# TobiasDeBruijn/UU-INFOGR-Raytracer

Hardware: AMD Instinct MI355X
Metric: Mray/s (primary+shadow+reflect) and fps at 1920×1080, 1/2/4/8 MI355X (higher is better)
Workload: dtype f32

## Files before the change

uu-infogr-raytracer_amd/csrc/rt_internal.h:

```cpp
#pragma once
#include <stdint.h>

#include "rt_resolve.h"

namespace rtk {

struct DevSphere {
    float cx, cy, cz, r2;
};

enum : uint32_t { MAT_MIRROR = 1u, MAT_DIFFUSE = 2u, MAT_SPEC = 4u, MAT_DARK_OK = 8u };

enum : uint32_t { POW_GENERIC = 0u, POW_ONE = 1u, POW_HALF = 2u, POW_TWO = 3u };

struct DevMaterial {
    float kd[3];
    float amb[3];
    float ks[3];
    float n;
    float km[3];
    uint32_t flags;
    uint32_t pow_kind;
    uint32_t pad;
};
// ... 80 lines not shown

struct CopyJob {
    const int32_t* src;
    int32_t* dst;
    unsigned long long words;
    unsigned long long dst_stride;
    unsigned band_words;
    unsigned pad;
};

struct alignas(16) DevView {
    float cam[3], right[3], up[3], fwd[3];
    int prim_const;
    int mbox_n;
    int mbox_plane[2];
    float mbox_tmax[2];
    int pad[2];
    PrimConst pc[MAX_PRIM_CONST];
    PrimBox pbox[MAX_PRIM_CONST];
    PrimBox mbox[2][CULL_MIN_SPHERES];
};
static_assert(sizeof(DevView) % 16 == 0, "DevView records are 16-byte aligned in their device table");

struct LaunchParams {
    const DevSphere* sph;
    const DevMaterial* mat;
    const DevPlane* pl;
    const DevLight* li;
    const DevSphereCull* scull;
    const DevShadowCull* shcull;
    const DevShadowCull* shpre;
    const DevShadowGrid* shg;
    const unsigned long long* shgrid;
    const unsigned long long* shslab;
    const DevCluster* clus;
    const float* lxt;
    const float* lyt;
    int S, P, L, limit;
    int lights_a2_ok;
    int n_clus;
    float cam[3], right[3], up[3], fwd[3];
    float pw, ph, nearc;
    int W, H;
    int band_rows, band_first, band_step, local_rows;
    int n_frames;
    int32_t* out;
    unsigned long long out_frame_bytes;
    int out_fmt;
    unsigned char* enc_wire;
    uint32_t* enc_stage;
    int enc_tiles_x, enc_tpf, enc_frame0;
    unsigned long long* counters;
    CopyJob copy;
    int copy_z;
    int prim_const;
    PrimConst pc[MAX_PRIM_CONST];
    PrimBox pbox[MAX_PRIM_CONST];
    int row_order_n;
    int col_major;
    uint16_t row_order[ROW_ORDER_MAX];
    const uint32_t* tile_order;
    uint32_t* tile_cost;
    int ss_log2;
    int mbox_n;
    int mbox_plane[2];
    float mbox_tmax[2];
    PrimBox mbox[2][CULL_MIN_SPHERES];
    const DevView* views;
    int shutter_log2;
    int adapt_thr;
    int foot_n;
    PlaneFoot foot[FOOT_MAX];
    ResolveSum* prog_acc;
    int prog_first;
    int prog_n;
    int prog_pass[2];
    int uniform_plane;
    const DevShadowGroups* shgrp;
    unsigned long long scene_stride;
    int view_ss;
};
constexpr int MIRROR_BOX_PLANES = 2;
constexpr int SINGLE_WPG = 4;
static_assert(sizeof(LaunchParams) < 4096, "LaunchParams is passed by value as the kernarg block (< 4 KiB)");

constexpr int OUT_TILES = 3;

constexpr int DIRECT_SMAX = 8;

enum : int { TV_DIRECT = 0, TV_BUNDLE = 1 };
enum : int { TM_PLAIN = 0, TM_STATS = 1, TM_TILES = 2, TM_SS = 3, TM_PATH = 4, TM_SHUTTER = 5, TM_ADAPT = 6, TM_PROG = 7, TM_ANIM = 8,
             TM_PATH_SS = 9, TM_SHUTTER_SS = 10, TM_ANIM_SS = 11 };
struct TraceVariant {
    int family;
    int gpow;
    int mode;
    int cls;
    int K;
    int wpg;
    int tord;
};

enum : unsigned { VF_GPOW = 1u, VF_STATS = 2u, VF_TILES = 4u, VF_SS = 8u, VF_PATH = 16u, VF_SHUTTER = 32u, VF_ADAPT = 64u, VF_PROG = 128u };
constexpr unsigned VF_ANIM = 1u << 18;
// ... 102 lines not shown
```

uu-infogr-raytracer_amd/csrc/rt_kernel.hip:

```cpp
#include <hip/hip_runtime.h>

#include "rt_fastmath.h"
#include "rt_codec_common.h"
#include "rt_dark.h"
#include "rt_foot.h"
#include "rt_internal.h"
#include "rt_pow.h"
#include "rt_prims.h"
#include "rt_resolve.h"
#include "rt_shadow_pre.h"

constexpr int WG_THREADS = 64, TILE_W = 8, TILE_H = 8;

namespace rtk {

constexpr unsigned COPY_WAVES = 512;
__device__ __forceinline__ size_t band_dst(const CopyJob& j, unsigned i) {
    if (j.band_words == 0) return i;
    const unsigned k = i / j.band_words;
    return (size_t)k * j.dst_stride + (i - k * j.band_words);
}
__device__ __forceinline__ void copy_job(const CopyJob& j, size_t wg, size_t nwg) {
    const size_t lane = threadIdx.x & 63;
    const unsigned long long n = j.words, n4 = n / 4;
// ... 7 lines not shown
            d4[i] = a;
            d4[i + step] = b;
            d4[i + 2 * step] = c;
            d4[i + 3 * step] = d;
        }
        for (; i < n4; i += step) d4[i] = s4[i];
    } else {
        int4* __restrict__ d4 = (int4*)j.dst;
        const unsigned bq = j.band_words / 4, sq = (unsigned)(j.dst_stride / 4);
        for (unsigned c = (unsigned)i; c < (unsigned)n4; c += (unsigned)step) {
            const unsigned k = c / bq;
            d4[k * sq + (c - k * bq)] = s4[c];
        }
    }
    if (wg == 0 && lane < n - n4 * 4) j.dst[band_dst(j, (unsigned)(n4 * 4 + lane))] = j.src[n4 * 4 + lane];
}
__device__ __forceinline__ void copy_slice(const LaunchParams& p) {
    const size_t nwg = min((size_t)gridDim.x * gridDim.y, (size_t)COPY_WAVES);
    const size_t wg = (size_t)blockIdx.y * gridDim.x + blockIdx.x;
    if (wg < nwg) copy_job(p.copy, wg, nwg);
}
__global__ __launch_bounds__(64) void band_copy_kernel(CopyJob j) { copy_job(j, blockIdx.x, gridDim.x); }

__device__ __forceinline__ void store_at(const LaunchParams& p, size_t i, uint32_t px32) {
    unsigned char* base = (unsigned char*)p.out + (size_t)blockIdx.z * p.out_frame_bytes;
    if (p.out_fmt != 1) {
        ((int32_t*)base)[i] = (int32_t)px32;
    } else {
        unsigned char* o = base + i * 3;
        o[0] = (unsigned char)px32;
        o[1] = (unsigned char)(px32 >> 8);
        o[2] = (unsigned char)(px32 >> 16);
    }
}
__device__ __forceinline__ void store_pixel(const LaunchParams& p, int r, int y, int x, uint32_t px32) {
    store_at(p, (size_t)(p.out_fmt == 2 ? y : r) * (size_t)p.W + (size_t)x, px32);
}

template <int CTRL>
__device__ __forceinline__ ResolveSum resolve_add_dpp(ResolveSum v) {
    return resolve_add(v, ResolveSum{(uint32_t)__builtin_amdgcn_update_dpp(0, (int)v.rb, CTRL, 0xf, 0xf, false),
                                     (uint32_t)__builtin_amdgcn_update_dpp(0, (int)v.g, CTRL, 0xf, 0xf, false)});
}
template <int PATTERN>
__device__ __forceinline__ ResolveSum resolve_add_swizzle(ResolveSum v) {
    return resolve_add(v, ResolveSum{(uint32_t)__builtin_amdgcn_ds_swizzle((int)v.rb, PATTERN),
                                     (uint32_t)__builtin_amdgcn_ds_swizzle((int)v.g, PATTERN)});
}
__device__ __forceinline__ ResolveSum resolve_block_sum(ResolveSum v, int s) {
    v = resolve_add_dpp<0xb1>(v);
    v = resolve_add_dpp<0x128>(v);
    if (s >= 2) {
        v = resolve_add_dpp<0x4e>(v);
        v = resolve_add_swizzle<0x401f>(v);
    }
    if (s >= 3) {
        v = resolve_add_swizzle<0x101f>(v);
        v = resolve_add(v, ResolveSum{(uint32_t)__shfl_xor((int)v.rb, 32, 64), (uint32_t)__shfl_xor((int)v.g, 32, 64)});
// ... 90 lines not shown
        if constexpr (PATH != VIEW_ARGS) return v().pc;
        else return p.pc;
    }
    __device__ __forceinline__ const PrimBox* pbox() const {
        if constexpr (PATH != VIEW_ARGS) return v().pbox;
        else return p.pbox;
    }
    __device__ __forceinline__ int mbox_n() const {
        if constexpr (PATH != VIEW_ARGS) return v().mbox_n;
        else return p.mbox_n;
    }
    __device__ __forceinline__ int mbox_plane(int k) const {
        if constexpr (PATH != VIEW_ARGS) return v().mbox_plane[k];
        else return p.mbox_plane[k];
    }
    __device__ __forceinline__ float mbox_tmax(int k) const {
        if constexpr (PATH != VIEW_ARGS) return v().mbox_tmax[k];
        else return p.mbox_tmax[k];
    }
    __device__ __forceinline__ const PrimBox* mbox(int k) const {
        if constexpr (PATH != VIEW_ARGS) return v().mbox[k];
        else return p.mbox[k];
    }
    __device__ __forceinline__ int foot_n() const {
        if constexpr (PATH != VIEW_ARGS) return -1;
        else return p.foot_n;
    }
};

template <int PATH>
struct SceneOf {
    template <bool NULLABLE, typename T>
    static __device__ __forceinline__ const T* at(const LaunchParams& p, const T* q) {
        if constexpr (PATH == VIEW_ANIM) {
            const T* z = (const T*)((const char*)q + (size_t)blockIdx.z * (size_t)p.scene_stride);
            if constexpr (NULLABLE) return q == nullptr ? nullptr : z;
            else return z;
        } else {
            return q;
        }
    }
    static __device__ __forceinline__ const DevSphere* sph(const LaunchParams& p) { return at<false>(p, p.sph); }
    static __device__ __forceinline__ const DevMaterial* mat(const LaunchParams& p) { return at<false>(p, p.mat); }
    static __device__ __forceinline__ const DevPlane* pl(const LaunchParams& p) { return at<false>(p, p.pl); }
    static __device__ __forceinline__ const DevLight* li(const LaunchParams& p) { return at<false>(p, p.li); }
    static __device__ __forceinline__ const DevSphereCull* scull(const LaunchParams& p) { return at<false>(p, p.scull); }
    static __device__ __forceinline__ const DevShadowCull* shcull(const LaunchParams& p) { return at<true>(p, p.shcull); }
    static __device__ __forceinline__ const DevShadowCull* shpre(const LaunchParams& p) { return at<true>(p, p.shpre); }
    static __device__ __forceinline__ const DevShadowGrid* shg(const LaunchParams& p) { return at<true>(p, p.shg); }
    static __device__ __forceinline__ const unsigned long long* shgrid(const LaunchParams& p) { return at<true>(p, p.shgrid); }
// ... 140 lines not shown
    static constexpr int smax = SMAX;
    unsigned s = 0, pl = 0, sh = 0;
    int lvl = 0, sel_cat = 0, sel_lvl = -1;
    __device__ __forceinline__ void sphere(bool c) { s += (!RT_SHADOW_CAT && (RT_SLOT_TALLY || c)) ? 1u : 0u; }
    __device__ __forceinline__ void shadow_sphere(bool c) {
        s += (!RT_SHADOW_CAT && (RT_SLOT_TALLY == 1 || c)) ? 1u : 0u;
    }
    __device__ __forceinline__ void plane(bool c) { pl += c ? 1u : 0u; }
    __device__ __forceinline__ void shadow(bool c) { sh += c ? 1u : 0u; }
    __device__ __forceinline__ void init(const LaunchParams& p) {
        sel_cat = p.enc_frame0 / 16;
        sel_lvl = p.enc_frame0 % 16 - 1;
    }
    __device__ __forceinline__ void set_level(int l) { lvl = l; }
    __device__ __forceinline__ void shadow_cat(int cat, unsigned n) {
        s += (RT_SHADOW_CAT && cat + 1 == sel_cat && (sel_lvl < 0 || lvl == sel_lvl)) ? n : 0u;
    }
    __device__ __forceinline__ void shadow_masks(int cat, unsigned long long m) {
        if (RT_SHADOW_CAT && cat + 1 == sel_cat && (sel_lvl < 0 || lvl == sel_lvl) && (threadIdx.x & 63) == 0)
            s += (unsigned)__builtin_popcountll(m);
    }
};

template <bool ST, int PATH = VIEW_ARGS, int SM>
__device__ __forceinline__ void add_counters(const LaunchParams& p, int lane, unsigned n_refl, unsigned n_shadow,
                                             const Tally<ST, SM>& tl) {
    if ((!PATH && blockIdx.z != (unsigned)p.copy_z) || p.counters == nullptr) return;
    const unsigned long long nf = !PATH && p.n_frames > 1 ? (unsigned long long)p.n_frames : 1ull;
    const unsigned b = wave_count(n_refl), c = wave_count(n_shadow);
    const unsigned slot = (blockIdx.y * gridDim.x + blockIdx.x) % COUNTER_SLOTS;
    unsigned long long* q = &p.counters[slot * COUNTER_STRIDE];
    if (lane == 0) {
        if (b) atomicAdd(q + CNT_REFLECT, b * nf);
        if (c) atomicAdd(q + CNT_SHADOW, c * nf);
    }
    if constexpr (ST) {
        const unsigned s = wave_count(tl.s), pl = wave_count(tl.pl), sh = wave_count(tl.sh);
        if (lane == 0) {
            if (sh) atomicAdd(q + CNT_SHADOW_RUN, sh * nf);
            if (s) atomicAdd(q + CNT_SPHERE_RUN, s * nf);
            if (pl) atomicAdd(q + CNT_PLANE_RUN, pl * nf);
        }
    }
}

#ifndef RT_UNIFORM_PLANE
#define RT_UNIFORM_PLANE 1
#endif
// ... 126 lines not shown
                tl.shadow(true);
                blocked = l_ok ? shadow_scan<true, GROUPS, PATH>(p, hp, l, li, tl) : shadow_scan<false, false, PATH>(p, hp, l, li, tl);
            }
            const float inten = blocked ? 0.0f : l.intensity;
            const float ia = inten * att;
            f3 term = mul(mk(ia, ia, ia), ph);
            if (!is_sphere) {
                term = mul(term, mk(tile, tile, tile));
                term = mk(nmax0(term.x), nmax0(term.y), nmax0(term.z));
            }
            col = add(col, term);
        }
    }
    if (flags & MAT_DIFFUSE) *n_shadow += (unsigned)p.L << CNT_SHADOW_SHIFT;
    return add(col, mk(m.amb[0], m.amb[1], m.amb[2]));
}

template <int PATH, typename T>
__device__ __forceinline__ f3 shade_plane_uniform(const LaunchParams& p, int plane, f3 hp, f3 d, float t, f3 sec,
                                                  unsigned* n_shadow, T& tl) {
    return shade_direct<false, RT_SHADOW_GROUPS != 0, PATH>(p, false, plane, hp, d, t, sec, n_shadow, tl);
}

__device__ __forceinline__ unsigned long long box_mask(const LaunchParams& p, const PrimBox* tab, int x, int y) {
    const int x_lo = __builtin_amdgcn_readlane(x, 0), x_hi = __builtin_amdgcn_readlane(x, 63);
    const int y_lo = __builtin_amdgcn_readlane(y, 0), y_hi = __builtin_amdgcn_readlane(y, 63);
    const int lane = threadIdx.x & 63;
    const bool in = lane < p.S;
    const PrimBox b = tab[in ? lane : 0];
    const bool cand = in & (b.x0 <= x_hi) & (b.x1 >= x_lo) & (b.y0 <= y_hi) & (b.y1 >= y_lo);
    return __builtin_amdgcn_ballot_w64(cand);
}
template <int PATH = VIEW_ARGS>
__device__ __forceinline__ unsigned long long prim_box_mask(const LaunchParams& p, int x, int y, int rec = 0) {
    return box_mask(p, ViewOf<PATH>{p, rec}.pbox(), x, y);
}
template <int PATH = VIEW_ARGS>
__device__ __forceinline__ unsigned mirror_box_masks(const LaunchParams& p, int x, int y, int rec = 0) {
    const ViewOf<PATH> vw{p, rec};
    unsigned m = 0;
    if (vw.mbox_n() > 0) {
        m = (unsigned)box_mask(p, vw.mbox(0), x, y);
        if (vw.mbox_n() > 1) m |= (unsigned)box_mask(p, vw.mbox(1), x, y) << 16;
    }
    return m;
}
template <int PATH = VIEW_ARGS>
__device__ __forceinline__ unsigned mirror_box_select(const LaunchParams& p, unsigned masks, float t, int prim, int rec = 0) {
    const ViewOf<PATH> vw{p, rec};
    const int pi = ~prim;
    const bool on0 = prim < 0 && pi == vw.mbox_plane(0) && t <= vw.mbox_tmax(0);
    const bool on1 = prim < 0 && pi == vw.mbox_plane(1) && t <= vw.mbox_tmax(1);
    if (__builtin_amdgcn_ballot_w64(!(on0 || on1)) != 0) return ~0u;
    unsigned m = 0;
    if (__builtin_amdgcn_ballot_w64(on0) != 0) m |= masks & 0xffffu;
    if (__builtin_amdgcn_ballot_w64(on1) != 0) m |= masks >> 16;
    return m;
}

struct TilePixel {
    int x, r, y;
    bool valid;
    float lx, ly;
};
template <bool SS = false>
__device__ __forceinline__ TilePixel tile_pixel(const LaunchParams& p, int x, int r) {
    TilePixel t;
    t.x = x, t.r = r;
    if (p.band_rows >= p.local_rows) {
        t.y = p.band_first * p.band_rows + r;
    } else if (!SS && p.band_rows == 8) {
        t.y = (p.band_first + (r >> 3) * p.band_step) * 8 + (r & 7);
    } else if (SS && (p.band_rows & (p.band_rows - 1)) == 0) {
        const int sh = 31 - __builtin_clz((unsigned)p.band_rows);
        t.y = ((p.band_first + (r >> sh) * p.band_step) << sh) + (r & (p.band_rows - 1));
    } else {
        const int band = p.band_first + (r / p.band_rows) * p.band_step;
        t.y = band * p.band_rows + (r % p.band_rows);
    }
    t.valid = x < p.W && r < p.local_rows && t.y < p.H;
    const float lx = p.lxt[t.valid ? x : 0], ly = p.lyt[t.valid ? t.y : 0];
    t.lx = t.valid ? lx : 0.0f, t.ly = t.valid ? ly : 0.0f;
    return t;
}
__device__ __forceinline__ TilePixel sample_pixel(const LaunchParams& p, int tile_x, int tile_y, int lane, int pass) {
    const int x = tile_x * TILE_W + (lane & 7), r = tile_y * TILE_H + (lane >> 3), s2 = p.ss_log2;
    return tile_pixel<true>(p, (x << s2) | (pass & ((1 << s2) - 1)), (r << s2) | (pass >> s2));
}

template <bool PRIMARY, bool A2OK, bool GATED, int PATH, typename T>
__device__ __forceinline__ void nearest_spheres(const LaunchParams& p, f3 o, f3 d, float a2, float a4, bool a2_ok,
                                                unsigned long long pmask, float& best_s, int& win_s, T& tl, int rec = 0) {
    if (PRIMARY && ViewOf<PATH>{p, rec}.prim_const()) {
        for (unsigned long long m = pmask; m;) {
            const int i = (int)__builtin_ctzll(m);
            m &= ~(1ull << i);
            tl.sphere(true);
            const PrimConst pc = ViewOf<PATH>{p, rec}.pc()[i];
            const float b = 2.0f * dot(mk(pc.ocx, pc.ocy, pc.ocz), d);
            const float disc = b * b - a4 * pc.c;
            const float t = A2OK ? root_t1(b, disc, a2) : (a2_ok ? root_t1(b, disc, a2) : root_full(b, disc, a2));
            take_primary(t, i, best_s, win_s);
        }
    } else {
        for_sphere_pairs<T>(p, [&](int i) {
            if constexpr (GATED) {
                if ((((unsigned)pmask >> i) & 3u) == 0) return;
            }
            tl.sphere(true);
            tl.sphere(i + 1 < p.S);
// ... 37 lines not shown
template <int PATH, typename T>
__device__ __forceinline__ Hit terminal_direct(const LaunchParams& p, f3 o, f3 d, T& tl) {
    float best_p = __builtin_inff();
    int win_p = -1;
    for (int i = 0; i < p.P; ++i) {
        tl.plane(true);
        plane_take(o, d, SceneOf<PATH>::pl(p)[i], i, best_p, win_p);
    }
    if (win_p < 0 || !(best_p - 0.01f > 0.0f)) return Hit{0.0f, HIT_NONE};
    const float a = dot(d, d);
    const float a2 = 2.0f * a, a4 = 4.0f * a;
    const bool a2_ok = a2 > 0.0f && a2 < __builtin_inff();
    float best_s = __builtin_inff();
    int win_s = -1;
    if (__builtin_amdgcn_ballot_w64(!a2_ok) == 0)
        nearest_spheres<false, true, false, PATH>(p, o, d, a2, a4, a2_ok, 0, best_s, win_s, tl);
    else
        nearest_spheres<false, false, false, PATH>(p, o, d, a2, a4, a2_ok, 0, best_s, win_s, tl);
    if (best_s < best_p) return Hit{0.0f, HIT_NONE};
    return Hit{best_p, ~win_p};
}

template <int PATH>
__device__ __forceinline__ bool sky_tile(const LaunchParams& p, const TilePixel& t, unsigned long long pmask, int rec) {
    const ViewOf<PATH> vw{p, rec};
    const int n = vw.foot_n();
    if (n < 0 || pmask != 0 || !vw.prim_const()) return false;
    bool may = false;
#pragma unroll
    for (int i = 0; i < FOOT_MAX; ++i) {
        if (i >= n) break;
        may |= foot_may_hit(p.foot[i], t.lx, t.ly);
    }
    return __builtin_amdgcn_ballot_w64(t.valid && may) == 0;
}

constexpr unsigned VF_TILE = ~(vf_wpg(15) | vf_tord(3));

struct TileOut {
    unsigned cnt;
    uint32_t px32;
};

template <int K, unsigned V, bool UNIFORM_OK = true, typename T>
__device__ __forceinline__ TileOut trace_tile_direct(const LaunchParams& p, int tile_x, int tile_y, float2* stk_lv,
                                                     float* stk_dv, T& tl, int rec = 0) {
    constexpr bool GPOW = (V & VF_GPOW) != 0, TILES = (V & VF_TILES) != 0, SS = ss_of(V), SHUTTER = shutter_of(V);
    constexpr bool ADAPT = (V & VF_ADAPT) != 0;
    constexpr int PATH = view_of(V);
    constexpr bool UNIFORM = RT_UNIFORM_PLANE && UNIFORM_OK && !GPOW;
    const int lane = threadIdx.x & 63;
    const TilePixel tpx = ADAPT ? sample_pixel(p, tile_x, tile_y, lane, rec)
                                : tile_pixel<SS>(p, tile_x * TILE_W + (lane & 7), tile_y * TILE_H + (lane >> 3));
    const int x = tpx.x, r = tpx.r, y = tpx.y;
    const bool valid = tpx.valid;
    const ViewOf<PATH> vw{p, rec};
    const unsigned long long pmask = vw.prim_const() ? prim_box_mask<PATH>(p, x, y, rec) : 0;
    const bool sky = sky_tile<PATH>(p, tpx, pmask, rec);
    unsigned mmask = 0;
    if constexpr (K > 1) {
        if (!sky) mmask = mirror_box_masks<PATH>(p, x, y, rec);
    }

    unsigned cnt = 0;
    typename StackFor<K>::type stk(stk_lv, stk_dv);
    f3 leaf = mk(0.0f, 0.0f, 0.0f);
    uint32_t px32 = 0;
    if (valid) {
        if (!sky) {
            const f3 cam = vw.cam();
            const float lx = tpx.lx, ly = tpx.ly, lz = 1.0f * p.nearc;
            const f3 vp = add(add(add(cam, scale(vw.right(), lx)), scale(vw.up(), ly)), scale(vw.fwd(), lz));
            f3 d = normalize(sub(vp, cam));
            f3 o = cam;

            stk.origin(d);
            Hit h = nearest_direct<true, false, PATH>(p, o, d, tl, pmask, rec);
            int count = 0;
            for (;;) {
                if (h.prim == HIT_NONE) break;
                if (h.t - 0.01f <= 0.0f) break;
                const bool is_sphere = h.prim >= 0;
                if (count > p.limit) {
                    if (!is_sphere) leaf = mk(1.0f, 1.0f, 1.0f);
// ... 24 lines not shown
                    const int code0 = __builtin_amdgcn_readlane(code, (int)__builtin_ctzll(m0));
                    if (code0 < 0 && __builtin_amdgcn_ballot_w64(rec0 && code != code0) == 0) floor_n = 1;
                }
            }
            f3 col = leaf;
            while (stk.n > floor_n) {
                float4 ra, rb;
                stk.template pop<PATH>(p, ra, rb, rec);
                const int code = __float_as_int(rb.w);
                const bool is_s = code >= 0;
                col = shade_direct<GPOW, false, PATH>(p, is_s, is_s ? code : ~code, mk(ra.x, ra.y, ra.z),
                                               mk(rb.x, rb.y, rb.z), ra.w, col, &cnt, tl);
            }
            if constexpr (UNIFORM) {
                if (floor_n != 0 && stk.n != 0) {
                    float4 ra, rb;
                    stk.template level0<PATH>(p, ra, rb, rec);
                    const int plane = ~__builtin_amdgcn_readfirstlane(__float_as_int(rb.w));
                    col = shade_plane_uniform<PATH>(p, plane, mk(ra.x, ra.y, ra.z), mk(rb.x, rb.y, rb.z), ra.w, col, &cnt, tl);
                }
            }
            px32 = (shift_channel(col.x) << 16) | (shift_channel(col.y) << 8) | shift_channel(col.z);
        }
        if constexpr (!TILES && !SS && !SHUTTER && !ADAPT) store_pixel(p, r, y, x, px32);
    }
    if constexpr (TILES) encode_tile_fused(p, px32, valid);
    if constexpr (SS && !SHUTTER) resolve_tile(p, r, y, x, valid, px32);
    return TileOut{cnt, px32};
}

template <bool SS, typename F>
__device__ __forceinline__ void shutter_tile(const LaunchParams& p, int tile_x, int tile_y, F trace) {
    const int t = p.shutter_log2, m = 1 << t;
    const int rec0 = (int)(blockIdx.z << t);
    const bool counting = p.counters != nullptr;
    ResolveSum acc{0u, 0u};
    unsigned long long n_refl = 0, n_shadow = 0;
#pragma unroll 1
    for (int s = 0; s < m; ++s) {
        int tx = tile_x, ty = tile_y;
        asm("" : "+s"(tx), "+s"(ty) : "s"(s));
        const __attribute__((address_space(4))) LaunchParams* kp =
            (const __attribute__((address_space(4))) LaunchParams*)__builtin_amdgcn_kernarg_segment_ptr();
        asm("" : "+s"(kp) : "s"(s));
        const TileOut o = trace(*(const LaunchParams*)kp, rec0 | s, tx, ty);
        acc = resolve_add(acc, resolve_unpack(o.px32));
        if (counting) {
            n_refl += wave_count(o.cnt & CNT_REFL_MASK);
            n_shadow += wave_count(o.cnt >> CNT_SHADOW_SHIFT);
        }
    }
// ... 91 lines not shown
        uint2* a = (uint2*)(p.prog_acc + ((size_t)(t.r >> s2) * wo + xo));
        if (p.prog_first > 0) {
            const uint2 before = *a;
            acc = resolve_add(acc, ResolveSum{before.x, before.y});
        }
        if (p.prog_n > 0) *a = make_uint2(acc.rb, acc.g);
        store_at(p, (size_t)((p.out_fmt == 2 ? t.y : t.r) >> s2) * wo + xo, resolve_round_div(acc, p.prog_first + p.prog_n));
    }
    if (p.counters != nullptr && blockIdx.z == (unsigned)p.copy_z && ln == 0) {
        unsigned long long* c = &p.counters[((blockIdx.y * gridDim.x + blockIdx.x) % COUNTER_SLOTS) * COUNTER_STRIDE];
        if (n_refl) atomicAdd(c + CNT_REFLECT, (unsigned long long)n_refl);
        if (n_shadow) atomicAdd(c + CNT_SHADOW, n_shadow);
    }
}

template <int K, unsigned V>
__device__ __forceinline__ void direct_kernel_body(const LaunchParams& p) {
    constexpr bool STATS = (V & VF_STATS) != 0, SHUTTER = shutter_of(V);
    constexpr int PATH = view_of(V);
    constexpr int SMAX = vf_cls_of(V), WPG = vf_wpg_of(V), TORD = vf_tord_of(V);
    constexpr int LDS_LEVELS = StackFor<K>::lds_levels;
    __shared__ float2 stk_lv[LDS_LEVELS > 0 ? LDS_LEVELS * WG_THREADS * WPG : 1];
    __shared__ float stk_dv[LDS_LEVELS > 0 ? 3 * WG_THREADS * WPG : 1];
    if (WPG == 1 && blockIdx.z < (unsigned)p.copy_z) {
        copy_slice(p);
        return;
    }
    Tally<STATS, SMAX> tl;
    const int wave = WPG > 1 && TORD != 0 ? __builtin_amdgcn_readfirstlane((int)(threadIdx.x >> 6))
                     : WPG > 1                ? (int)(threadIdx.x >> 6)
                                              : 0;
    float2* lv = stk_lv + (LDS_LEVELS > 0 ? wave * LDS_LEVELS * WG_THREADS : 0);
    float* dv = stk_dv + (LDS_LEVELS > 0 ? wave * 3 * WG_THREADS : 0);
    const bool cm = WPG > 1 && p.col_major;
    const int gx = cm ? (int)blockIdx.y : (int)blockIdx.x, gy = cm ? (int)blockIdx.x : (int)blockIdx.y;
    int tile_x = gx * WPG + wave, tile_y = WPG > 1 && gy < p.row_order_n ? (int)p.row_order[gy] : gy;
    if constexpr (TORD == 1) {
        const uint32_t t = p.tile_order[blockIdx.x * WPG + wave];
        tile_x = (int)(t & 0xffffu), tile_y = (int)(t >> 16);
    }
    struct TileRec {
        unsigned* slot;
        unsigned t0;
    };
    __shared__ TileRec t_rec[TORD == 2 ? WPG : 1];
    if (TORD == 2 && (threadIdx.x & 63) == 0) {
        const unsigned tiles_x = (unsigned)(p.W + TILE_W - 1) / TILE_W, tiles_y = (unsigned)(p.H + TILE_H - 1) / TILE_H;
        const bool in = p.tile_cost != nullptr && (unsigned)tile_x < tiles_x && (unsigned)tile_y < tiles_y;
        t_rec[wave] = TileRec{in ? p.tile_cost + ((unsigned)tile_y * tiles_x + (unsigned)tile_x) : nullptr,
                              in ? (unsigned)__builtin_amdgcn_s_memrealtime() : 0u};
    }
    if constexpr (SHUTTER) {
        shutter_tile<ss_of(V)>(p, tile_x, tile_y, [&](const LaunchParams& q, int rec, int tx, int ty) { return trace_tile_direct<K, V & VF_TILE>(q, tx, ty, lv, dv, tl, rec); });
        return;
    }
    if constexpr ((V & VF_ADAPT) != 0) {
        adaptive_tile(p, tile_x, tile_y, [&](const LaunchParams& q, int pass, int tx, int ty) { return trace_tile_direct<K, V & VF_TILE>(q, tx, ty, lv, dv, tl, pass); });
        return;
    }
    if constexpr ((V & VF_PROG) != 0) {
        progressive_tile(p, tile_x, tile_y, [&](const LaunchParams& q, int pass, int tx, int ty) { return trace_tile_direct<K, ((V & VF_TILE) & ~VF_PROG) | VF_ADAPT>(q, tx, ty, lv, dv, tl, pass); });
        return;
    }
    const unsigned cnt = trace_tile_direct<K, V & VF_TILE, TORD != 2>(p, tile_x, tile_y, lv, dv, tl).cnt;
    add_counters<STATS, PATH>(p, threadIdx.x & 63, cnt & CNT_REFL_MASK, cnt >> CNT_SHADOW_SHIFT, tl);
    if (TORD == 2 && (threadIdx.x & 63) == 0) {
        const TileRec r = t_rec[threadIdx.x >> 6];
        if (r.slot != nullptr) *r.slot = (unsigned)__builtin_amdgcn_s_memrealtime() - r.t0;
    }
}
template <int K, unsigned V>
__global__ __launch_bounds__(WG_THREADS * vf_wpg_of(V)) __attribute__((amdgpu_num_sgpr(80))) void trace_direct_kernel(LaunchParams p) {
    static_assert(!(V & VF_GPOW), "GPOW variants run trace_direct_kernel_gpow");
    direct_kernel_body<K, V>(p);
}
template <int K, unsigned V>
__global__ __launch_bounds__(WG_THREADS * vf_wpg_of(V)) void trace_direct_kernel_gpow(LaunchParams p) {
    static_assert((V & VF_GPOW) != 0, "variants without GPOW run trace_direct_kernel");
    direct_kernel_body<K, V>(p);
}

struct Bundle {
    f3 O, A;
    float R, delta;
    bool ok;
    bool any;
};

__device__ __forceinline__ float readlane_f(float v, int lane) {
    return __int_as_float(__builtin_amdgcn_readlane(__float_as_int(v), lane));
}
__device__ __forceinline__ f3 readlane3(f3 v, int lane) {
    return mk(readlane_f(v.x, lane), readlane_f(v.y, lane), readlane_f(v.z, lane));
}
template <int CTRL>
// ... 462 lines not shown
        float4 ra = make_float4(0.0f, 0.0f, 0.0f, 1.0f), rb = make_float4(0.0f, 0.0f, 1.0f, 0.0f);
        if (act) stk.template pop<PATH>(p, ra, rb, rec);
        const unsigned long long am = __builtin_amdgcn_ballot_w64(act);
        if (am != ~0ull) {
            const int ref = __builtin_ctzll(am);
            const float4 qa = make_float4(readlane_f(ra.x, ref), readlane_f(ra.y, ref), readlane_f(ra.z, ref),
                                          readlane_f(ra.w, ref));
            const float4 qb = make_float4(readlane_f(rb.x, ref), readlane_f(rb.y, ref), readlane_f(rb.z, ref),
                                          readlane_f(rb.w, ref));
            if (!act) {
                ra = qa;
                rb = qb;
            }
        }
        const int code = __float_as_int(rb.w);
        const bool is_s = code >= 0;
        tl.set_level(level);
        col = shade_bundle<GPOW, MERGED, PATH>(p, act, is_s, is_s ? code : ~code, mk(ra.x, ra.y, ra.z), mk(rb.x, rb.y, rb.z),
                                         ra.w, col, cnt, tl, level);
    }
    return col;
}

template <int K, unsigned V, typename T>
__device__ __forceinline__ TileOut trace_tile_bundle(const LaunchParams& p, int tile_x, int tile_y, float2* stk_lv,
                                                     float* stk_dv, T& tl, int rec = 0) {
    constexpr bool GPOW = (V & VF_GPOW) != 0, TILES = (V & VF_TILES) != 0, SS = ss_of(V), SHUTTER = shutter_of(V);
    constexpr bool ADAPT = (V & VF_ADAPT) != 0;
    constexpr int PATH = view_of(V);
    constexpr int MERGED = vf_cls_of(V);
    const int lane = threadIdx.x & 63;
    const TilePixel tpx = ADAPT ? sample_pixel(p, tile_x, tile_y, lane, rec)
                                : tile_pixel<SS>(p, tile_x * TILE_W + (lane & 7), tile_y * TILE_H + (lane >> 3));
    const int x = tpx.x, y = tpx.y;
    const bool valid = tpx.valid;

    unsigned cnt = 0;
    const ViewOf<PATH> vw{p, rec};
    const f3 cam = vw.cam();
    const float lx = tpx.lx, ly = tpx.ly, lz = 1.0f * p.nearc;
    const f3 vp = add(add(add(cam, scale(vw.right(), lx)), scale(vw.up(), ly)), scale(vw.fwd(), lz));
    f3 d = normalize(sub(vp, cam));
    f3 o = cam;

    typename StackFor<K>::type stk(stk_lv, stk_dv);
    stk.origin(d);
    f3 leaf = mk(0.0f, 0.0f, 0.0f);
    bool active = valid;
    const unsigned long long pmask = vw.prim_const() ? prim_box_mask<PATH>(p, x, y, rec) : 0;
    Hit h = nearest_bundle<true, PATH>(p, o, d, active, tl, pmask, nullptr, rec);
    for (int count = 0;; ++count) {
        if (active) {
            const bool is_sphere = h.prim >= 0;
            if (h.prim == HIT_NONE || h.t - 0.01f <= 0.0f) {
                active = false;
            } else if (count > p.limit) {
                if (!is_sphere) leaf = mk(1.0f, 1.0f, 1.0f);
                active = false;
            } else {
                const f3 hp = add(o, scale(d, h.t));
                stk.push(make_float4(hp.x, hp.y, hp.z, h.t), make_float4(d.x, d.y, d.z, __int_as_float(h.prim)));
                const int prim = is_sphere ? h.prim : ~h.prim;
                const uint32_t flags = SceneOf<PATH>::mat(p)[is_sphere ? prim : p.S + prim].flags;
                if (!(flags & MAT_MIRROR)) {
                    active = false;
                } else {
                    o = reflect_at<PATH>(p, o, d, h.t, h.prim);
                    ++cnt;
                }
            }
        }
        if (__builtin_amdgcn_ballot_w64(active) == 0) break;
// ... 16 lines not shown
        }
    }

    const f3 col = fold_converged<GPOW, MERGED, PATH>(p, stk, leaf, &cnt, tl, rec);
    const uint32_t px32 = (shift_channel(col.x) << 16) | (shift_channel(col.y) << 8) | shift_channel(col.z);
    if constexpr (TILES) encode_tile_fused(p, px32, valid);
    else if constexpr (!SHUTTER && !ADAPT) {
        const int ln = (int)__builtin_amdgcn_mbcnt_hi(~0u, __builtin_amdgcn_mbcnt_lo(~0u, 0u));
        const TilePixel q = tile_pixel<SS>(p, tile_x * TILE_W + (ln & 7), tile_y * TILE_H + (ln >> 3));
        if constexpr (SS) resolve_tile(p, q.r, q.y, q.x, q.valid, px32);
        else if (q.valid) store_pixel(p, q.r, q.y, q.x, px32);
    }
    return TileOut{cnt, px32};
}

template <int K, unsigned V>
__device__ __forceinline__ void bundle_kernel_body(const LaunchParams& p) {
    constexpr bool STATS = (V & VF_STATS) != 0, SHUTTER = shutter_of(V);
    constexpr int PATH = view_of(V);
    constexpr int TORD = vf_tord_of(V);
    constexpr int LDS_LEVELS = StackFor<K>::lds_levels;
    __shared__ float2 stk_lv[LDS_LEVELS > 0 ? LDS_LEVELS * WG_THREADS : 1];
    __shared__ float stk_dv[LDS_LEVELS > 0 ? 3 * WG_THREADS : 1];
    if (blockIdx.z < (unsigned)p.copy_z) {
        copy_slice(p);
        return;
    }
    Tally<STATS> tl;
    tl.init(p);
    int tile_x = (int)blockIdx.x, tile_y = (int)blockIdx.y;
    if constexpr (TORD == 1) {
        const uint32_t t = p.tile_order[blockIdx.y * gridDim.x + blockIdx.x];
        tile_x = (int)(t & 0xffffu), tile_y = (int)(t >> 16);
    }
    struct TileRec {
        unsigned* slot;
        unsigned t0;
    };
    __shared__ TileRec t_rec[1];
    if (TORD == 2 && (threadIdx.x & 63) == 0)
        t_rec[0] = TileRec{blockIdx.z == (unsigned)p.copy_z ? p.tile_cost + (blockIdx.y * gridDim.x + blockIdx.x) : nullptr,
                           (unsigned)__builtin_amdgcn_s_memrealtime()};
    if constexpr (SHUTTER) {
        shutter_tile<ss_of(V)>(p, tile_x, tile_y, [&](const LaunchParams& q, int rec, int tx, int ty) { return trace_tile_bundle<K, V & VF_TILE>(q, tx, ty, stk_lv, stk_dv, tl, rec); });
        return;
    }
    if constexpr ((V & VF_ADAPT) != 0) {
        adaptive_tile(p, tile_x, tile_y, [&](const LaunchParams& q, int pass, int tx, int ty) { return trace_tile_bundle<K, V & VF_TILE>(q, tx, ty, stk_lv, stk_dv, tl, pass); });
        return;
    }
    if constexpr ((V & VF_PROG) != 0) {
        progressive_tile(p, tile_x, tile_y, [&](const LaunchParams& q, int pass, int tx, int ty) { return trace_tile_bundle<K, ((V & VF_TILE) & ~VF_PROG) | VF_ADAPT>(q, tx, ty, stk_lv, stk_dv, tl, pass); });
        return;
    }
    const unsigned cnt = trace_tile_bundle<K, V & VF_TILE>(p, tile_x, tile_y, stk_lv, stk_dv, tl).cnt;
    add_counters<STATS, PATH>(p, threadIdx.x & 63, cnt & CNT_REFL_MASK, cnt >> CNT_SHADOW_SHIFT, tl);
    if (TORD == 2 && (threadIdx.x & 63) == 0 && t_rec[0].slot != nullptr)
        *t_rec[0].slot = (unsigned)__builtin_amdgcn_s_memrealtime() - t_rec[0].t0;
}
template <int K, unsigned V>
__global__ __launch_bounds__(WG_THREADS, 8) __attribute__((amdgpu_num_sgpr(80))) void trace_bundle_kernel(
    LaunchParams p) {
    static_assert(!(V & VF_GPOW), "GPOW variants run trace_bundle_kernel_gpow");
    bundle_kernel_body<K, V>(p);
}
template <int K, unsigned V>
__global__ __launch_bounds__(WG_THREADS) void trace_bundle_kernel_gpow(LaunchParams p) {
    static_assert((V & VF_GPOW) != 0, "variants without GPOW run trace_bundle_kernel");
    bundle_kernel_body<K, V>(p);
}

__device__ __forceinline__ void append_segment(DevSegment* out, int cap, unsigned* count, f3 o, f3 e, int kind,
                                               int pixel) {
    const unsigned i = atomicAdd(count, 1u);
    if (i < (unsigned)cap) out[i] = DevSegment{o.x, o.y, o.z, e.x, e.y, e.z, kind, pixel};
}

__global__ __launch_bounds__(256) void debug_segments_kernel(LaunchParams p, int stride, DevSegment* out, int cap,
// ... 178 lines not shown
```

Baseline: 305,700.

## Reorder kernel arguments into cache-line head and batch early scalar loads

Reorders LaunchParams so the per-wave scalars read at kernel entry (dimensions, band layout, counts, footprints) sit together in two 64-byte lines at offset 0, with the output tail grouped into one line. It also adds load_head and wave_tables helpers that pull these fields and the per-lane box tables into registers together at the start, using empty asm pins to keep them in SGPRs and VGPRs. The goal is fewer scattered, serialized kernarg scalar loads and an earlier issue of the lxt/lyt and box loads. In exchange it raises register pressure under the 80-SGPR cap, and it adds an optional tail path that is off by default.

```diff
diff --git a/uu-infogr-raytracer_amd/csrc/rt_internal.h b/uu-infogr-raytracer_amd/csrc/rt_internal.h
--- a/uu-infogr-raytracer_amd/csrc/rt_internal.h
+++ b/uu-infogr-raytracer_amd/csrc/rt_internal.h
@@ -1,5 +1,7 @@
 #pragma once
 #include <stdint.h>
+
+#include <type_traits>
 
 #include "rt_resolve.h"
 
@@ -126,7 +128,43 @@
 };
 static_assert(sizeof(DevView) % 16 == 0, "DevView records are 16-byte aligned in their device table");
 
-struct LaunchParams {
+struct alignas(64) LaunchHead {
+    const float* lxt;
+    const float* lyt;
+    int W, H;
+    int band_rows, band_first, band_step, local_rows;
+    int ss_log2;
+    int copy_z;
+    int prim_const;
+    int S;
+    int foot_n;
+    int mbox_n;
+    int P, L, limit;
+    int uniform_plane;
+    int mbox_plane[2];
+    float mbox_tmax[2];
+    const DevView* views;
+    int row_order_n;
+    int col_major;
+    int lights_a2_ok;
+    int n_clus;
+    int head_pad[2];
+};
+static_assert(sizeof(LaunchHead) == 128 && alignof(LaunchHead) == 64, "the launch head is two 64-byte lines");
+
+struct LaunchParams : LaunchHead {
+    PlaneFoot foot[FOOT_MAX];
+    float pw, ph, nearc;
+    int tail_pad;
+    int32_t* out;
+    unsigned long long out_frame_bytes;
+    unsigned long long* counters;
+    unsigned char* enc_wire;
+    uint32_t* enc_stage;
+    int out_fmt;
+    int n_frames;
+    int enc_tiles_x, enc_tpf, enc_frame0;
+    int tail_end_pad;
     const DevSphere* sph;
     const DevMaterial* mat;
     const DevPlane* pl;
@@ -138,52 +176,46 @@
     const unsigned long long* shgrid;
     const unsigned long long* shslab;
     const DevCluster* clus;
-    const float* lxt;
-    const float* lyt;
-    int S, P, L, limit;
-    int lights_a2_ok;
-    int n_clus;
     float cam[3], right[3], up[3], fwd[3];
-    float pw, ph, nearc;
-    int W, H;
-    int band_rows, band_first, band_step, local_rows;
-    int n_frames;
-    int32_t* out;
-    unsigned long long out_frame_bytes;
-    int out_fmt;
-    unsigned char* enc_wire;
-    uint32_t* enc_stage;
-    int enc_tiles_x, enc_tpf, enc_frame0;
-    unsigned long long* counters;
     CopyJob copy;
-    int copy_z;
-    int prim_const;
     PrimConst pc[MAX_PRIM_CONST];
     PrimBox pbox[MAX_PRIM_CONST];
-    int row_order_n;
-    int col_major;
+    PrimBox mbox[2][CULL_MIN_SPHERES];
     uint16_t row_order[ROW_ORDER_MAX];
     const uint32_t* tile_order;
     uint32_t* tile_cost;
-    int ss_log2;
-    int mbox_n;
-    int mbox_plane[2];
-    float mbox_tmax[2];
-    PrimBox mbox[2][CULL_MIN_SPHERES];
-    const DevView* views;
+    int line_pad[10];
     int shutter_log2;
     int adapt_thr;
-    int foot_n;
-    PlaneFoot foot[FOOT_MAX];
     ResolveSum* prog_acc;
     int prog_first;
     int prog_n;
     int prog_pass[2];
-    int uniform_plane;
     const DevShadowGroups* shgrp;
     unsigned long long scene_stride;
     int view_ss;
 };
+static_assert(std::is_trivially_copyable<LaunchParams>::value && std::is_base_of<LaunchHead, LaunchParams>::value,
+              "LaunchParams is copied into the kernel argument segment byte for byte");
+#if defined(__clang__)
+#pragma clang diagnostic push
+#pragma clang diagnostic ignored "-Winvalid-offsetof"
+#elif defined(__GNUC__)
+#pragma GCC diagnostic push
+#pragma GCC diagnostic ignored "-Winvalid-offsetof"
+#endif
+static_assert(__builtin_offsetof(LaunchParams, view_ss) + 2 * sizeof(int) == sizeof(LaunchParams), "view_ss is the last word");
+static_assert(alignof(LaunchParams) == 64 && __builtin_offsetof(LaunchParams, lxt) == 0 &&
+                  __builtin_offsetof(LaunchParams, foot) == sizeof(LaunchHead),
+              "the launch head at offset 0, the plane footprints directly behind it");
+static_assert(__builtin_offsetof(LaunchParams, out) % 64 == 0 &&
+                  __builtin_offsetof(LaunchParams, enc_frame0) + sizeof(int) <= __builtin_offsetof(LaunchParams, out) + 64,
+              "the tail: one 64-byte line");
+#if defined(__clang__)
+#pragma clang diagnostic pop
+#elif defined(__GNUC__)
+#pragma GCC diagnostic pop
+#endif
 constexpr int MIRROR_BOX_PLANES = 2;
 constexpr int SINGLE_WPG = 4;
 static_assert(sizeof(LaunchParams) < 4096, "LaunchParams is passed by value as the kernarg block (< 4 KiB)");
diff --git a/uu-infogr-raytracer_amd/csrc/rt_kernel.hip b/uu-infogr-raytracer_amd/csrc/rt_kernel.hip
--- a/uu-infogr-raytracer_amd/csrc/rt_kernel.hip
+++ b/uu-infogr-raytracer_amd/csrc/rt_kernel.hip
@@ -53,7 +53,8 @@
 }
 __global__ __launch_bounds__(64) void band_copy_kernel(CopyJob j) { copy_job(j, blockIdx.x, gridDim.x); }
 
-__device__ __forceinline__ void store_at(const LaunchParams& p, size_t i, uint32_t px32) {
+template <typename O>
+__device__ __forceinline__ void store_at(const O& p, size_t i, uint32_t px32) {
     unsigned char* base = (unsigned char*)p.out + (size_t)blockIdx.z * p.out_frame_bytes;
     if (p.out_fmt != 1) {
         ((int32_t*)base)[i] = (int32_t)px32;
@@ -64,7 +65,8 @@
         o[2] = (unsigned char)(px32 >> 16);
     }
 }
-__device__ __forceinline__ void store_pixel(const LaunchParams& p, int r, int y, int x, uint32_t px32) {
+template <typename O>
+__device__ __forceinline__ void store_pixel(const O& p, int r, int y, int x, uint32_t px32) {
     store_at(p, (size_t)(p.out_fmt == 2 ? y : r) * (size_t)p.W + (size_t)x, px32);
 }
 
@@ -201,10 +203,6 @@
         if constexpr (PATH != VIEW_ARGS) return v().mbox[k];
         else return p.mbox[k];
     }
-    __device__ __forceinline__ int foot_n() const {
-        if constexpr (PATH != VIEW_ARGS) return -1;
-        else return p.foot_n;
-    }
 };
 
 template <int PATH>
@@ -391,8 +389,8 @@
     }
 };
 
-template <bool ST, int PATH = VIEW_ARGS, int SM>
-__device__ __forceinline__ void add_counters(const LaunchParams& p, int lane, unsigned n_refl, unsigned n_shadow,
+template <bool ST, int PATH = VIEW_ARGS, int SM, typename O>
+__device__ __forceinline__ void add_counters(const O& p, int lane, unsigned n_refl, unsigned n_shadow,
                                              const Tally<ST, SM>& tl) {
     if ((!PATH && blockIdx.z != (unsigned)p.copy_z) || p.counters == nullptr) return;
     const unsigned long long nf = !PATH && p.n_frames > 1 ? (unsigned long long)p.n_frames : 1ull;
@@ -565,26 +563,29 @@
     return shade_direct<false, RT_SHADOW_GROUPS != 0, PATH>(p, false, plane, hp, d, t, sec, n_shadow, tl);
 }
 
-__device__ __forceinline__ unsigned long long box_mask(const LaunchParams& p, const PrimBox* tab, int x, int y) {
+__device__ __forceinline__ PrimBox box_load(const PrimBox* tab, int S) {
+    const int lane = threadIdx.x & 63;
+    return tab[lane < S ? lane : 0];
+}
+__device__ __forceinline__ unsigned long long box_test(const PrimBox& b, int S, int x, int y) {
     const int x_lo = __builtin_amdgcn_readlane(x, 0), x_hi = __builtin_amdgcn_readlane(x, 63);
     const int y_lo = __builtin_amdgcn_readlane(y, 0), y_hi = __builtin_amdgcn_readlane(y, 63);
-    const int lane = threadIdx.x & 63;
-    const bool in = lane < p.S;
-    const PrimBox b = tab[in ? lane : 0];
+    const bool in = (int)(threadIdx.x & 63) < S;
     const bool cand = in & (b.x0 <= x_hi) & (b.x1 >= x_lo) & (b.y0 <= y_hi) & (b.y1 >= y_lo);
     return __builtin_amdgcn_ballot_w64(cand);
+}
+__device__ __forceinline__ unsigned long long box_mask(const LaunchHead& h, const PrimBox* tab, int x, int y) {
+    return box_test(box_load(tab, h.S), h.S, x, y);
 }
 template <int PATH = VIEW_ARGS>
 __device__ __forceinline__ unsigned long long prim_box_mask(const LaunchParams& p, int x, int y, int rec = 0) {
     return box_mask(p, ViewOf<PATH>{p, rec}.pbox(), x, y);
 }
-template <int PATH = VIEW_ARGS>
-__device__ __forceinline__ unsigned mirror_box_masks(const LaunchParams& p, int x, int y, int rec = 0) {
-    const ViewOf<PATH> vw{p, rec};
+__device__ __forceinline__ unsigned mirror_box_masks(const PrimBox& b0, const PrimBox& b1, int mbox_n, int S, int x, int y) {
     unsigned m = 0;
-    if (vw.mbox_n() > 0) {
-        m = (unsigned)box_mask(p, vw.mbox(0), x, y);
-        if (vw.mbox_n() > 1) m |= (unsigned)box_mask(p, vw.mbox(1), x, y) << 16;
+    if (mbox_n > 0) {
+        m = (unsigned)box_test(b0, S, x, y);
+        if (mbox_n > 1) m |= (unsigned)box_test(b1, S, x, y) << 16;
     }
     return m;
 }
@@ -607,7 +608,7 @@
     float lx, ly;
 };
 template <bool SS = false>
-__device__ __forceinline__ TilePixel tile_pixel(const LaunchParams& p, int x, int r) {
+__device__ __forceinline__ TilePixel tile_pixel(const LaunchHead& p, int x, int r) {
     TilePixel t;
     t.x = x, t.r = r;
     if (p.band_rows >= p.local_rows) {
@@ -622,13 +623,79 @@
         t.y = band * p.band_rows + (r % p.band_rows);
     }
     t.valid = x < p.W && r < p.local_rows && t.y < p.H;
-    const float lx = p.lxt[t.valid ? x : 0], ly = p.lyt[t.valid ? t.y : 0];
+    typedef const __attribute__((address_space(1))) float* gtab;
+    const float lx = ((gtab)p.lxt)[t.valid ? x : 0], ly = ((gtab)p.lyt)[t.valid ? t.y : 0];
     t.lx = t.valid ? lx : 0.0f, t.ly = t.valid ? ly : 0.0f;
     return t;
 }
-__device__ __forceinline__ TilePixel sample_pixel(const LaunchParams& p, int tile_x, int tile_y, int lane, int pass) {
+__device__ __forceinline__ TilePixel sample_pixel(const LaunchHead& p, int tile_x, int tile_y, int lane, int pass) {
     const int x = tile_x * TILE_W + (lane & 7), r = tile_y * TILE_H + (lane >> 3), s2 = p.ss_log2;
     return tile_pixel<true>(p, (x << s2) | (pass & ((1 << s2) - 1)), (r << s2) | (pass >> s2));
+}
+
+struct WaveHead : LaunchHead {
+    PlaneFoot foot[FOOT_MAX];
+};
+template <bool FOOT>
+__device__ __forceinline__ WaveHead load_head(int tie = 0) {
+    const __attribute__((address_space(4))) LaunchParams* kp =
+        (const __attribute__((address_space(4))) LaunchParams*)__builtin_amdgcn_kernarg_segment_ptr();
+    asm("" : "+s"(kp) : "s"(tie));
+    const LaunchParams& p = *(const LaunchParams*)kp;
+    WaveHead h;
+    static_cast<LaunchHead&>(h) = p;
+    if constexpr (FOOT) {
+#pragma unroll
+        for (int i = 0; i < FOOT_MAX; ++i) h.foot[i] = p.foot[i];
+        asm("" : "+s"(h.lxt), "+s"(h.lyt), "+s"(h.W), "+s"(h.H), "+s"(h.band_rows), "+s"(h.band_first), "+s"(h.band_step),
+                 "+s"(h.local_rows), "+s"(h.ss_log2), "+s"(h.copy_z), "+s"(h.prim_const), "+s"(h.S), "+s"(h.foot_n), "+s"(h.mbox_n),
+                 "+s"(h.foot[0].a), "+s"(h.foot[0].b), "+s"(h.foot[0].c), "+s"(h.foot[1].a), "+s"(h.foot[1].b), "+s"(h.foot[1].c),
+                 "+s"(h.foot[2].a), "+s"(h.foot[2].b), "+s"(h.foot[2].c), "+s"(h.foot[3].a), "+s"(h.foot[3].b), "+s"(h.foot[3].c));
+    } else {
+        asm("" : "+s"(h.lxt), "+s"(h.lyt), "+s"(h.W), "+s"(h.H), "+s"(h.band_rows), "+s"(h.band_first), "+s"(h.band_step),
+                 "+s"(h.local_rows), "+s"(h.ss_log2), "+s"(h.copy_z), "+s"(h.prim_const), "+s"(h.S), "+s"(h.foot_n), "+s"(h.mbox_n));
+    }
+    return h;
+}
+#ifndef RT_TAIL_ROUND
+#define RT_TAIL_ROUND 0
+#endif
+constexpr bool direct_tail_of(unsigned V) {
+    return RT_TAIL_ROUND && (V & (VF_TILES | VF_ADAPT | VF_PROG)) == 0 && !ss_of(V) && !shutter_of(V);
+}
+struct WaveTail {
+    int32_t* out;
+    unsigned long long out_frame_bytes;
+    unsigned long long* counters;
+    int out_fmt, n_frames, W, copy_z;
+};
+__device__ __forceinline__ WaveTail load_tail(uint32_t px32) {
+    const __attribute__((address_space(4))) LaunchParams* kp =
+        (const __attribute__((address_space(4))) LaunchParams*)__builtin_amdgcn_kernarg_segment_ptr();
+    asm("" : "+s"(kp) : "v"(px32));
+    const LaunchParams& p = *(const LaunchParams*)kp;
+    WaveTail t{p.out, p.out_frame_bytes, p.counters, p.out_fmt, p.n_frames, p.W, p.copy_z};
+    asm("" : "+s"(t.out), "+s"(t.out_frame_bytes), "+s"(t.counters), "+s"(t.out_fmt), "+s"(t.n_frames), "+s"(t.W), "+s"(t.copy_z));
+    return t;
+}
+struct WaveTables {
+    PrimBox pbox, mbox0, mbox1;
+};
+template <int PATH, bool MIRROR>
+__device__ __forceinline__ WaveTables wave_tables(const LaunchParams& p, const LaunchHead& h, TilePixel& t, int rec) {
+    const ViewOf<PATH> vw{p, rec};
+    WaveTables w{};
+    w.pbox = box_load(vw.pbox(), h.S);
+    if constexpr (MIRROR) {
+        w.mbox0 = box_load(vw.mbox(0), h.S);
+        w.mbox1 = box_load(vw.mbox(1), h.S);
+        asm("" : "+v"(t.lx), "+v"(t.ly), "+v"(w.pbox.x0), "+v"(w.pbox.x1), "+v"(w.pbox.y0), "+v"(w.pbox.y1),
+                 "+v"(w.mbox0.x0), "+v"(w.mbox0.x1), "+v"(w.mbox0.y0), "+v"(w.mbox0.y1),
+                 "+v"(w.mbox1.x0), "+v"(w.mbox1.x1), "+v"(w.mbox1.y0), "+v"(w.mbox1.y1));
+    } else {
+        asm("" : "+v"(t.lx), "+v"(t.ly), "+v"(w.pbox.x0), "+v"(w.pbox.x1), "+v"(w.pbox.y0), "+v"(w.pbox.y1));
+    }
+    return w;
 }
 
 template <bool PRIMARY, bool A2OK, bool GATED, int PATH, typename T>
@@ -712,15 +779,15 @@
 }
 
 template <int PATH>
-__device__ __forceinline__ bool sky_tile(const LaunchParams& p, const TilePixel& t, unsigned long long pmask, int rec) {
-    const ViewOf<PATH> vw{p, rec};
-    const int n = vw.foot_n();
-    if (n < 0 || pmask != 0 || !vw.prim_const()) return false;
+__device__ __forceinline__ bool sky_tile(const WaveHead& h, const TilePixel& t, unsigned long long pmask) {
+    if constexpr (PATH != VIEW_ARGS) return false;
+    const int n = h.foot_n;
+    if (n < 0 || pmask != 0 || !h.prim_const) return false;
     bool may = false;
 #pragma unroll
     for (int i = 0; i < FOOT_MAX; ++i) {
         if (i >= n) break;
-        may |= foot_may_hit(p.foot[i], t.lx, t.ly);
+        may |= foot_may_hit(h.foot[i], t.lx, t.ly);
     }
     return __builtin_amdgcn_ballot_w64(t.valid && may) == 0;
 }
@@ -730,26 +797,30 @@
 struct TileOut {
     unsigned cnt;
     uint32_t px32;
+    WaveTail tail;
 };
 
 template <int K, unsigned V, bool UNIFORM_OK = true, typename T>
-__device__ __forceinline__ TileOut trace_tile_direct(const LaunchParams& p, int tile_x, int tile_y, float2* stk_lv,
-                                                     float* stk_dv, T& tl, int rec = 0) {
+__device__ __forceinline__ TileOut trace_tile_direct(const LaunchParams& p, const WaveHead& hd, int tile_x, int tile_y,
+                                                     float2* stk_lv, float* stk_dv, T& tl, int rec = 0) {
     constexpr bool GPOW = (V & VF_GPOW) != 0, TILES = (V & VF_TILES) != 0, SS = ss_of(V), SHUTTER = shutter_of(V);
     constexpr bool ADAPT = (V & VF_ADAPT) != 0;
     constexpr int PATH = view_of(V);
+    constexpr bool TAIL = direct_tail_of(V);
     constexpr bool UNIFORM = RT_UNIFORM_PLANE && UNIFORM_OK && !GPOW;
     const int lane = threadIdx.x & 63;
-    const TilePixel tpx = ADAPT ? sample_pixel(p, tile_x, tile_y, lane, rec)
-                                : tile_pixel<SS>(p, tile_x * TILE_W + (lane & 7), tile_y * TILE_H + (lane >> 3));
+    TilePixel tpx = ADAPT ? sample_pixel(hd, tile_x, tile_y, lane, rec)
+                          : tile_pixel<SS>(hd, tile_x * TILE_W + (lane & 7), tile_y * TILE_H + (lane >> 3));
+    const WaveTables wt = wave_tables<PATH, (K > 1)>(p, hd, tpx, rec);
     const int x = tpx.x, r = tpx.r, y = tpx.y;
     const bool valid = tpx.valid;
     const ViewOf<PATH> vw{p, rec};
-    const unsigned long long pmask = vw.prim_const() ? prim_box_mask<PATH>(p, x, y, rec) : 0;
-    const bool sky = sky_tile<PATH>(p, tpx, pmask, rec);
+    const int prim_const = PATH == VIEW_ARGS ? hd.prim_const : vw.prim_const();
+    const unsigned long long pmask = prim_const ? box_test(wt.pbox, hd.S, x, y) : 0;
+    const bool sky = sky_tile<PATH>(hd, tpx, pmask);
     unsigned mmask = 0;
     if constexpr (K > 1) {
-        if (!sky) mmask = mirror_box_masks<PATH>(p, x, y, rec);
+        if (!sky) mmask = mirror_box_masks(wt.mbox0, wt.mbox1, PATH == VIEW_ARGS ? hd.mbox_n : vw.mbox_n(), hd.S, x, y);
     }
 
     unsigned cnt = 0;
@@ -820,11 +891,16 @@
             }
             px32 = (shift_channel(col.x) << 16) | (shift_channel(col.y) << 8) | shift_channel(col.z);
         }
-        if constexpr (!TILES && !SS && !SHUTTER && !ADAPT) store_pixel(p, r, y, x, px32);
+        if constexpr (!TAIL && !TILES && !SS && !SHUTTER && !ADAPT) store_pixel(p, r, y, x, px32);
+    }
+    WaveTail tail{};
+    if constexpr (TAIL) {
+        tail = load_tail(px32);
+        if (valid) store_pixel(tail, r, y, x, px32);
     }
     if constexpr (TILES) encode_tile_fused(p, px32, valid);
     if constexpr (SS && !SHUTTER) resolve_tile(p, r, y, x, valid, px32);
-    return TileOut{cnt, px32};
+    return TileOut{cnt, px32, tail};
 }
 
 template <bool SS, typename F>
@@ -962,7 +1038,11 @@
     constexpr int LDS_LEVELS = StackFor<K>::lds_levels;
     __shared__ float2 stk_lv[LDS_LEVELS > 0 ? LDS_LEVELS * WG_THREADS * WPG : 1];
     __shared__ float stk_dv[LDS_LEVELS > 0 ? 3 * WG_THREADS * WPG : 1];
-    if (WPG == 1 && blockIdx.z < (unsigned)p.copy_z) {
+    constexpr bool LOOPS = SHUTTER || (V & (VF_ADAPT | VF_PROG)) != 0;
+    WaveHead hd{};
+    if constexpr (LOOPS) hd.copy_z = p.copy_z;
+    else hd = load_head<PATH == VIEW_ARGS>();
+    if (WPG == 1 && blockIdx.z < (unsigned)hd.copy_z) {
         copy_slice(p);
         return;
     }
@@ -991,26 +1071,31 @@
                               in ? (unsigned)__builtin_amdgcn_s_memrealtime() : 0u};
     }
     if constexpr (SHUTTER) {
-        shutter_tile<ss_of(V)>(p, tile_x, tile_y, [&](const LaunchParams& q, int rec, int tx, int ty) { return trace_tile_direct<K, V & VF_TILE>(q, tx, ty, lv, dv, tl, rec); });
+        shutter_tile<ss_of(V)>(p, tile_x, tile_y, [&](const LaunchParams& q, int rec, int tx, int ty) { return trace_tile_direct<K, V & VF_TILE>(q, load_head<false>(rec), tx, ty, lv, dv, tl, rec); });
         return;
     }
     if constexpr ((V & VF_ADAPT) != 0) {
-        adaptive_tile(p, tile_x, tile_y, [&](const LaunchParams& q, int pass, int tx, int ty) { return trace_tile_direct<K, V & VF_TILE>(q, tx, ty, lv, dv, tl, pass); });
+        adaptive_tile(p, tile_x, tile_y, [&](const LaunchParams& q, int pass, int tx, int ty) { return trace_tile_direct<K, V & VF_TILE>(q, load_head<true>(pass), tx, ty, lv, dv, tl, pass); });
         return;
     }
     if constexpr ((V & VF_PROG) != 0) {
-        progressive_tile(p, tile_x, tile_y, [&](const LaunchParams& q, int pass, int tx, int ty) { return trace_tile_direct<K, ((V & VF_TILE) & ~VF_PROG) | VF_ADAPT>(q, tx, ty, lv, dv, tl, pass); });
+        progressive_tile(p, tile_x, tile_y, [&](const LaunchParams& q, int pass, int tx, int ty) { return trace_tile_direct<K, ((V & VF_TILE) & ~VF_PROG) | VF_ADAPT>(q, load_head<true>(pass), tx, ty, lv, dv, tl, pass); });
         return;
     }
-    const unsigned cnt = trace_tile_direct<K, V & VF_TILE, TORD != 2>(p, tile_x, tile_y, lv, dv, tl).cnt;
-    add_counters<STATS, PATH>(p, threadIdx.x & 63, cnt & CNT_REFL_MASK, cnt >> CNT_SHADOW_SHIFT, tl);
+    const TileOut to = trace_tile_direct<K, V & VF_TILE, TORD != 2>(p, hd, tile_x, tile_y, lv, dv, tl);
+    const unsigned cnt = to.cnt;
+    if constexpr (direct_tail_of(V)) add_counters<STATS, PATH>(to.tail, threadIdx.x & 63, cnt & CNT_REFL_MASK, cnt >> CNT_SHADOW_SHIFT, tl);
+    else add_counters<STATS, PATH>(p, threadIdx.x & 63, cnt & CNT_REFL_MASK, cnt >> CNT_SHADOW_SHIFT, tl);
     if (TORD == 2 && (threadIdx.x & 63) == 0) {
         const TileRec r = t_rec[threadIdx.x >> 6];
         if (r.slot != nullptr) *r.slot = (unsigned)__builtin_amdgcn_s_memrealtime() - r.t0;
     }
 }
+#ifndef RT_DIRECT_SGPR_CAP
+#define RT_DIRECT_SGPR_CAP 80
+#endif
 template <int K, unsigned V>
-__global__ __launch_bounds__(WG_THREADS * vf_wpg_of(V)) __attribute__((amdgpu_num_sgpr(80))) void trace_direct_kernel(LaunchParams p) {
+__global__ __launch_bounds__(WG_THREADS * vf_wpg_of(V)) __attribute__((amdgpu_num_sgpr(RT_DIRECT_SGPR_CAP))) void trace_direct_kernel(LaunchParams p) {
     static_assert(!(V & VF_GPOW), "GPOW variants run trace_direct_kernel_gpow");
     direct_kernel_body<K, V>(p);
 }
@@ -1519,16 +1604,29 @@
     return col;
 }
 
+#ifndef RT_BUNDLE_HEAD
+#define RT_BUNDLE_HEAD 1
+#endif
+__device__ __forceinline__ WaveHead bundle_head(int tie) {
+    if constexpr (RT_BUNDLE_HEAD) return load_head<false>(tie);
+    else return WaveHead{};
+}
 template <int K, unsigned V, typename T>
-__device__ __forceinline__ TileOut trace_tile_bundle(const LaunchParams& p, int tile_x, int tile_y, float2* stk_lv,
-                                                     float* stk_dv, T& tl, int rec = 0) {
+__device__ __forceinline__ TileOut trace_tile_bundle(const LaunchParams& p, const WaveHead& hd, int tile_x, int tile_y,
+                                                     float2* stk_lv, float* stk_dv, T& tl, int rec = 0) {
     constexpr bool GPOW = (V & VF_GPOW) != 0, TILES = (V & VF_TILES) != 0, SS = ss_of(V), SHUTTER = shutter_of(V);
     constexpr bool ADAPT = (V & VF_ADAPT) != 0;
     constexpr int PATH = view_of(V);
     constexpr int MERGED = vf_cls_of(V);
     const int lane = threadIdx.x & 63;
+#if RT_BUNDLE_HEAD
+    TilePixel tpx = ADAPT ? sample_pixel(hd, tile_x, tile_y, lane, rec)
+                          : tile_pixel<SS>(hd, tile_x * TILE_W + (lane & 7), tile_y * TILE_H + (lane >> 3));
+    const WaveTables wt = wave_tables<PATH, false>(p, hd, tpx, rec);
+#else
     const TilePixel tpx = ADAPT ? sample_pixel(p, tile_x, tile_y, lane, rec)
                                 : tile_pixel<SS>(p, tile_x * TILE_W + (lane & 7), tile_y * TILE_H + (lane >> 3));
+#endif
     const int x = tpx.x, y = tpx.y;
     const bool valid = tpx.valid;
 
@@ -1544,7 +1642,11 @@
     stk.origin(d);
     f3 leaf = mk(0.0f, 0.0f, 0.0f);
     bool active = valid;
+#if RT_BUNDLE_HEAD
+    const unsigned long long pmask = (PATH == VIEW_ARGS ? hd.prim_const : vw.prim_const()) ? box_test(wt.pbox, hd.S, x, y) : 0;
+#else
     const unsigned long long pmask = vw.prim_const() ? prim_box_mask<PATH>(p, x, y, rec) : 0;
+#endif
     Hit h = nearest_bundle<true, PATH>(p, o, d, active, tl, pmask, nullptr, rec);
     for (int count = 0;; ++count) {
         if (active) {
@@ -1607,7 +1709,11 @@
     constexpr int LDS_LEVELS = StackFor<K>::lds_levels;
     __shared__ float2 stk_lv[LDS_LEVELS > 0 ? LDS_LEVELS * WG_THREADS : 1];
     __shared__ float stk_dv[LDS_LEVELS > 0 ? 3 * WG_THREADS : 1];
-    if (blockIdx.z < (unsigned)p.copy_z) {
+    constexpr bool LOOPS = SHUTTER || (V & (VF_ADAPT | VF_PROG)) != 0;
+    WaveHead hd{};
+    if constexpr (LOOPS || !RT_BUNDLE_HEAD) hd.copy_z = p.copy_z;
+    else hd = load_head<false>();
+    if (blockIdx.z < (unsigned)hd.copy_z) {
         copy_slice(p);
         return;
     }
@@ -1627,18 +1733,18 @@
         t_rec[0] = TileRec{blockIdx.z == (unsigned)p.copy_z ? p.tile_cost + (blockIdx.y * gridDim.x + blockIdx.x) : nullptr,
                            (unsigned)__builtin_amdgcn_s_memrealtime()};
     if constexpr (SHUTTER) {
-        shutter_tile<ss_of(V)>(p, tile_x, tile_y, [&](const LaunchParams& q, int rec, int tx, int ty) { return trace_tile_bundle<K, V & VF_TILE>(q, tx, ty, stk_lv, stk_dv, tl, rec); });
+        shutter_tile<ss_of(V)>(p, tile_x, tile_y, [&](const LaunchParams& q, int rec, int tx, int ty) { return trace_tile_bundle<K, V & VF_TILE>(q, bundle_head(rec), tx, ty, stk_lv, stk_dv, tl, rec); });
         return;
     }
     if constexpr ((V & VF_ADAPT) != 0) {
-        adaptive_tile(p, tile_x, tile_y, [&](const LaunchParams& q, int pass, int tx, int ty) { return trace_tile_bundle<K, V & VF_TILE>(q, tx, ty, stk_lv, stk_dv, tl, pass); });
+        adaptive_tile(p, tile_x, tile_y, [&](const LaunchParams& q, int pass, int tx, int ty) { return trace_tile_bundle<K, V & VF_TILE>(q, bundle_head(pass), tx, ty, stk_lv, stk_dv, tl, pass); });
         return;
     }
     if constexpr ((V & VF_PROG) != 0) {
-        progressive_tile(p, tile_x, tile_y, [&](const LaunchParams& q, int pass, int tx, int ty) { return trace_tile_bundle<K, ((V & VF_TILE) & ~VF_PROG) | VF_ADAPT>(q, tx, ty, stk_lv, stk_dv, tl, pass); });
+        progressive_tile(p, tile_x, tile_y, [&](const LaunchParams& q, int pass, int tx, int ty) { return trace_tile_bundle<K, ((V & VF_TILE) & ~VF_PROG) | VF_ADAPT>(q, bundle_head(pass), tx, ty, stk_lv, stk_dv, tl, pass); });
         return;
     }
-    const unsigned cnt = trace_tile_bundle<K, V & VF_TILE>(p, tile_x, tile_y, stk_lv, stk_dv, tl).cnt;
+    const unsigned cnt = trace_tile_bundle<K, V & VF_TILE>(p, hd, tile_x, tile_y, stk_lv, stk_dv, tl).cnt;
     add_counters<STATS, PATH>(p, threadIdx.x & 63, cnt & CNT_REFL_MASK, cnt >> CNT_SHADOW_SHIFT, tl);
     if (TORD == 2 && (threadIdx.x & 63) == 0 && t_rec[0].slot != nullptr)
         *t_rec[0].slot = (unsigned)__builtin_amdgcn_s_memrealtime() - t_rec[0].t0;
```

Measured after the change: 307,200 (median of 6 runs). About the same (+0.5%).
